# megvii-research/basedet

Hardware: AMD Instinct MI355X
Metric: images/sec training RetinaNet-R50-FPN 1333x800 (higher is better)
Workload: dtype bf16; 1 GPU; retinanet_r50_800x1344 train step (fwd+bwd+allreduce+SGD), DummyLoader boxes, random-init weights, inputs resident in HBM; per_gpu_batch=16, global_batch=16, parallelism=dp1

## Files before the change

### basedet_amd/csrc/gskip.hip

```cpp
#include "common.h"

namespace {

enum { GS_ANY = 1, GS_TOP = 2, GS_BOT = 4, GS_LEFT = 8, GS_RIGHT = 16, GS_TL = 32, GS_TR = 64, GS_BL = 128, GS_BR = 256 };

struct GsSeg { int patch_start, H, W, pw, off; };

struct GsParams {
    const bf16_raw* g;
    int* mask;
    int C, ppi, ph, pw_px, nseg, patches_per_img, total;
    GsSeg seg[BD_MAX_SEGS];
};

__device__ __forceinline__ int gs_level(const GsParams& p, int rem) {
    int s = 0;
#pragma unroll
    for (int k = 1; k < BD_MAX_SEGS; ++k)
        if (k < p.nseg && rem >= p.seg[k].patch_start) s = k;
    return s;
}

__global__ __launch_bounds__(256) void gskip_scan_kernel(const GsParams p) {
    __shared__ int sbits;
    const int tid = threadIdx.x;
    const int pid = blockIdx.x;
    const int n = pid / p.patches_per_img, rem = pid - n * p.patches_per_img;
    const int s = gs_level(p, rem);
    const int H = p.seg[s].H, W = p.seg[s].W, pwn = p.seg[s].pw;
    const int local = rem - p.seg[s].patch_start, by = local / pwn, bx = local - by * pwn;
    const int y0 = by * p.ph, x0 = bx * p.pw_px;
    const int cpp = p.C >> 3;
    const int items = p.ph * p.pw_px * cpp;
    const long long img = (long long)n * p.ppi + p.seg[s].off;
    if (tid == 0) sbits = 0;
    __syncthreads();
    int bits = 0;
    constexpr int U = 8;
    for (int b = 0; b < items; b += 256 * U) {
        u32x4_t v[U];
        int pix[U];
#pragma unroll
        for (int k = 0; k < U; ++k) {
            const int i = b + k * 256 + tid;
            v[k] = (u32x4_t){0u, 0u, 0u, 0u};
            pix[k] = -1;
            if (i < items) {
                const int px = i / cpp, ch = i - px * cpp;
                const int py = px / p.pw_px, pxx = px - py * p.pw_px;
                const int y = y0 + py, x = x0 + pxx;
                if (y < H && x < W) {
                    v[k] = *reinterpret_cast<const u32x4_t*>(p.g + (img + (long long)y * W + x) * p.C + ch * 8);
                    pix[k] = px;
                }
            }
        }
#pragma unroll
        for (int k = 0; k < U; ++k) {
            if (pix[k] >= 0 && (v[k][0] | v[k][1] | v[k][2] | v[k][3])) {
                const int py = pix[k] / p.pw_px, pxx = pix[k] - py * p.pw_px;
                const bool t = py == 0, bo = py == p.ph - 1, l = pxx == 0, r = pxx == p.pw_px - 1;
                bits |= GS_ANY | (t ? GS_TOP : 0) | (bo ? GS_BOT : 0) | (l ? GS_LEFT : 0) | (r ? GS_RIGHT : 0) | (t && l ? GS_TL : 0) |
                        (t && r ? GS_TR : 0) | (bo && l ? GS_BL : 0) | (bo && r ? GS_BR : 0);
            }
        }
    }
#pragma unroll
    for (int m = 32; m >= 1; m >>= 1) bits |= __shfl_xor(bits, m, 64);
    if ((tid & 63) == 0 && bits) atomicOr(&sbits, bits);
    __syncthreads();
    if (tid == 0) p.mask[pid] = sbits;
}

template <bool FRESH>
__device__ __forceinline__ int gs_mask(const int* m, int i) {
    if (FRESH) return __hip_atomic_load(m + i, __ATOMIC_RELAXED, __HIP_MEMORY_SCOPE_AGENT);
    return m[i];
}

template <bool FRESH>
__device__ __forceinline__ void gs_compact_body(const GsParams& p, int* live, int* list, int* count, int* wsum) {
    constexpr int KP = 8;
    const int tid = threadIdx.x, wv = tid >> 6, ln = tid & 63;
    int base = 0;
    for (int c0 = 0; c0 < p.total; c0 += 1024 * KP) {
        int lv[KP];
#pragma unroll
        for (int j = 0; j < KP; ++j) {
            const int q = c0 + tid * KP + j;
            lv[j] = 0;
            if (q < p.total) {
                const int n = q / p.patches_per_img, rem = q - n * p.patches_per_img;
                const int s = gs_level(p, rem);
                const int pwn = p.seg[s].pw, rows = (p.seg[s].H + p.ph - 1) / p.ph;
                const int local = rem - p.seg[s].patch_start, by = local / pwn, bx = local - by * pwn;
                const int* m = p.mask + (long long)n * p.patches_per_img + p.seg[s].patch_start;
                const bool up = by > 0, dn = by + 1 < rows, lf = bx > 0, rt = bx + 1 < pwn;
                int v = gs_mask<FRESH>(m, by * pwn + bx) & GS_ANY;
                if (up) v |= gs_mask<FRESH>(m, (by - 1) * pwn + bx) & GS_BOT;
                if (dn) v |= gs_mask<FRESH>(m, (by + 1) * pwn + bx) & GS_TOP;
                if (lf) v |= gs_mask<FRESH>(m, by * pwn + bx - 1) & GS_RIGHT;
                if (rt) v |= gs_mask<FRESH>(m, by * pwn + bx + 1) & GS_LEFT;
                if (up && lf) v |= gs_mask<FRESH>(m, (by - 1) * pwn + bx - 1) & GS_BR;
                if (up && rt) v |= gs_mask<FRESH>(m, (by - 1) * pwn + bx + 1) & GS_BL;
                if (dn && lf) v |= gs_mask<FRESH>(m, (by + 1) * pwn + bx - 1) & GS_TR;
                if (dn && rt) v |= gs_mask<FRESH>(m, (by + 1) * pwn + bx + 1) & GS_TL;
                lv[j] = v != 0;
            }
        }
        int cnt = 0;
#pragma unroll
        for (int j = 0; j < KP; ++j) cnt += lv[j];
        int inc = cnt;
#pragma unroll
        for (int o = 1; o < 64; o <<= 1) {
            const int y = __shfl_up(inc, o, 64);
            if (ln >= o) inc += y;
        }
        if (ln == 63) wsum[wv] = inc;
        __syncthreads();
        int off = base + inc - cnt, tot = 0;
#pragma unroll
        for (int w = 0; w < 16; ++w) {
            off += w < wv ? wsum[w] : 0;
            tot += wsum[w];
        }
#pragma unroll
        for (int j = 0; j < KP; ++j) {
            const int q = c0 + tid * KP + j;
            if (q < p.total) live[q] = lv[j];
            if (lv[j]) list[off++] = q;
        }
        base += tot;
        __syncthreads();
    }
    if (tid == 0) *count = base;
}

__global__ __launch_bounds__(1024) void gskip_compact_kernel(const GsParams p, int* live, int* list, int* count) {
    __shared__ int wsum[16];
    gs_compact_body<false>(p, live, list, count, wsum);
}

enum { GM_HDR = 8 };

struct GmSeg { int H, W, off, s4, s8, ss; };

struct GmParams {
    const bf16_raw* t;
    const int* live_in;
    int* map;
    int C, ppi, nseg, pi4, pi8, pis, tot4, tot8;
    GmSeg seg[BD_MAX_SEGS];
};

__global__ __launch_bounds__(1024) void gskip_fill_kernel(const GmParams p, const GsParams cp, int total) {
    __shared__ int sbits, slast;
    __shared__ int wsum[16];
    const int tid = threadIdx.x;
    int* m4 = p.map + GM_HDR;
    int* m8 = m4 + p.tot4;
    const int cpp = p.C >> 3;
    const int items = 4 * 16 * cpp;
    for (int pid = blockIdx.x; pid < total; pid += gridDim.x) {
        const int n = pid / p.pis, rem = pid - n * p.pis;
        int s = 0;
#pragma unroll
        for (int k = 1; k < BD_MAX_SEGS; ++k)
            if (k < p.nseg && rem >= p.seg[k].ss) s = k;
        const int H = p.seg[s].H, W = p.seg[s].W;
        const int sc = (W + 15) >> 4, r4 = (H + 3) >> 2, c8 = (W + 7) >> 3;
        const int local = rem - p.seg[s].ss, sy = local / sc, sx = local - sy * sc;
        int q4[2], q8[2];
        bool ok4[2], ok8[2], lv[2];
#pragma unroll
        for (int h = 0; h < 2; ++h) {
            ok4[h] = 2 * sy + h < r4;
            q4[h] = n * p.pi4 + p.seg[s].s4 + (2 * sy + h) * sc + sx;
            ok8[h] = 2 * sx + h < c8;
            q8[h] = n * p.pi8 + p.seg[s].s8 + sy * c8 + 2 * sx + h;
            lv[h] = ok4[h] && (p.live_in == nullptr || p.live_in[q4[h]] != 0);
        }
        int b = 0;
        if (lv[0] || lv[1]) {
            if (tid == 0) sbits = 0;
            __syncthreads();
            const long long img = (long long)n * p.ppi + p.seg[s].off;
            int bits = 0;
#pragma unroll
            for (int h = 0; h < 2; ++h) {
                if (!lv[h]) continue;
                for (int i = tid; i < items; i += 1024) {
                    const int px = i / cpp, ch = i - px * cpp;
                    const int py = px >> 4, pxx = px & 15;
                    const int y = 8 * sy + 4 * h + py, x = 16 * sx + pxx;
                    if (y < H && x < W) {
                        const u32x4_t v = *reinterpret_cast<const u32x4_t*>(p.t + (img + (long long)y * W + x) * p.C + ch * 8);
                        if (v[0] | v[1] | v[2] | v[3]) {
                            const bool t = py == 0, bo = py == 3, l = pxx == 0, r = pxx == 15;
                            const int w = GS_ANY | (t ? GS_TOP : 0) | (bo ? GS_BOT : 0) | (l ? GS_LEFT : 0) | (r ? GS_RIGHT : 0) |
                                          (t && l ? GS_TL : 0) | (t && r ? GS_TR : 0) | (bo && l ? GS_BL : 0) | (bo && r ? GS_BR : 0);
                            bits |= (w << (9 * h)) | (1 << (18 + (pxx >> 3)));
                        }
                    }
                }
            }
#pragma unroll
            for (int m = 32; m >= 1; m >>= 1) bits |= __shfl_xor(bits, m, 64);
            if ((tid & 63) == 0 && bits) atomicOr(&sbits, bits);
            __syncthreads();
            b = sbits;
            __syncthreads();
        }
        if (tid == 0) {
            if (ok4[0]) m4[q4[0]] = b & 511;
            if (ok4[1]) m4[q4[1]] = (b >> 9) & 511;
            if (ok8[0]) m8[q8[0]] = (b >> 18) & 1;
            if (ok8[1]) m8[q8[1]] = (b >> 19) & 1;
        }
    }
    if (tid == 0) {
        __builtin_amdgcn_fence(__ATOMIC_RELEASE, "agent");
        slast = atomicAdd(p.map + 1, 1) == (int)gridDim.x - 1;
    }
    __syncthreads();
    if (!slast) return;
    __builtin_amdgcn_fence(__ATOMIC_ACQUIRE, "agent");
    const int nxt = (p.map[0] & 1) ^ 1;
    int* live = m8 + p.tot8;
    gs_compact_body<true>(cp, live, live + p.tot4 * (1 + nxt), p.map + 2 + nxt, wsum);
    if (tid == 0) { p.map[0] = nxt; p.map[1] = 0; }
}

enum { FL_HDR = 8, FL_MAX_DEPTH = 8 };

struct FlSeg { int H, W, off, s4, pw; };

struct FlParams {
    const int* labels;
    int* map[FL_MAX_DEPTH];
    int A, ppi, nseg, depths, pi4, tot4;
    FlSeg seg[BD_MAX_SEGS];
};

__global__ __launch_bounds__(1024) void fwd_live_kernel(const FlParams p) {
    extern __shared__ __attribute__((aligned(16))) unsigned char fl_bm[];
    __shared__ int slast;
    __shared__ int wsum[16];
    const int tid = threadIdx.x;
    const int n = blockIdx.x / p.nseg, s = blockIdx.x - n * p.nseg;
    const int H = p.seg[s].H, W = p.seg[s].W, HW = H * W, pwn = p.seg[s].pw;
    const int npatch = ((H + 3) >> 2) * pwn;
    unsigned char* cur = fl_bm;
    unsigned char* nxt = fl_bm + HW;
    for (int i = tid; i < HW; i += 1024) cur[i] = 0;
    __syncthreads();
    const int* lab = p.labels + ((long long)n * p.ppi + p.seg[s].off) * p.A;
    for (int i = tid; i < HW * p.A; i += 1024)
        if (lab[i] > 0) cur[i / p.A] = 1;
    __syncthreads();
    for (int k = 0; k < p.depths; ++k) {
        for (int i = tid; i < HW; i += 1024) {
            const int y = i / W, x = i - y * W;
            const int y0 = y > 0 ? y - 1 : 0, y1 = y + 1 < H ? y + 1 : H - 1, x0 = x > 0 ? x - 1 : 0, x1 = x + 1 < W ? x + 1 : W - 1;
            int v = 0;
            for (int yy = y0; yy <= y1; ++yy)
                for (int xx = x0; xx <= x1; ++xx) v |= cur[yy * W + xx];
            nxt[i] = (unsigned char)v;
        }
        __syncthreads();
        int* live = p.map[k] + FL_HDR + n * p.pi4 + p.seg[s].s4;
        for (int q = tid; q < npatch; q += 1024) {
            const int by = q / pwn, bx = q - by * pwn;
            const int ye = by * 4 + 4 < H ? by * 4 + 4 : H, xe = bx * 16 + 16 < W ? bx * 16 + 16 : W;
            int v = 0;
            for (int y = by * 4; y < ye; ++y)
                for (int x = bx * 16; x < xe; ++x) v |= nxt[y * W + x];
            live[q] = v;
        }
        unsigned char* t = cur; cur = nxt; nxt = t;
        __syncthreads();
    }
    __builtin_amdgcn_fence(__ATOMIC_RELEASE, "agent");
    __syncthreads();
    if (tid == 0) slast = atomicAdd(p.map[0] + 1, 1) == (int)gridDim.x - 1;
    __syncthreads();
    if (!slast) return;
    __builtin_amdgcn_fence(__ATOMIC_ACQUIRE, "agent");
    constexpr int KP = 8;
    const int wv = tid >> 6, ln = tid & 63;
    for (int k = 0; k < p.depths; ++k) {
        int* hdr = p.map[k];
        const int* live = hdr + FL_HDR;
        const int to = (hdr[0] & 1) ^ 1;
        int* list = hdr + FL_HDR + p.tot4 * (1 + to);
        int base = 0;
        for (int c0 = 0; c0 < p.tot4; c0 += 1024 * KP) {
            int lv[KP];
            int cnt = 0;
#pragma unroll
            for (int j = 0; j < KP; ++j) {
                const int q = c0 + tid * KP + j;
                lv[j] = q < p.tot4 ? (__hip_atomic_load(live + q, __ATOMIC_RELAXED, __HIP_MEMORY_SCOPE_AGENT) != 0) : 0;
                cnt += lv[j];
            }
            int inc = cnt;
#pragma unroll
            for (int o = 1; o < 64; o <<= 1) {
                const int y = __shfl_up(inc, o, 64);
                if (ln >= o) inc += y;
            }
            if (ln == 63) wsum[wv] = inc;
            __syncthreads();
            int off = base + inc - cnt, tot = 0;
#pragma unroll
            for (int w = 0; w < 16; ++w) {
                off += w < wv ? wsum[w] : 0;
                tot += wsum[w];
            }
#pragma unroll
            for (int j = 0; j < KP; ++j)
                if (lv[j]) list[off++] = c0 + tid * KP + j;
            base += tot;
            __syncthreads();
        }
        if (tid == 0) { hdr[2 + to] = base; hdr[0] = to; }
    }
    if (tid == 0) p.map[0][1] = 0;
}

GsParams gs_params(const bd_conv_desc* d, int ph, int pw, int side = 0) {
    GsParams p{};
    p.C = side ? d->Cin : d->Cout; p.ppi = side ? d->in_pix_per_img : d->out_pix_per_img; p.ph = ph; p.pw_px = pw; p.nseg = d->nseg;
    int ps = 0;
    for (int s = 0; s < d->nseg; ++s) {
        GsSeg& sg = p.seg[s];
        const int H = side ? d->Hi[s] : d->Ho[s], W = side ? d->Wi[s] : d->Wo[s];
        sg.patch_start = ps; sg.H = H; sg.W = W; sg.pw = cdiv(W, pw); sg.off = side ? d->in_off[s] : d->out_off[s];
        ps += cdiv(H, ph) * sg.pw;
    }
    p.patches_per_img = ps;
    p.total = ps * d->N;
    return p;
}

}

int bd_gskip_patches(const bd_conv_desc* d, int ph, int pw) {
    return gs_params(d, ph, pw).total;
}

void bd_gskip_scan(const bd_conv_desc* d, const void* g, int ph, int pw, int* mask, hipStream_t stream) {
    GsParams p = gs_params(d, ph, pw);
    p.g = (const bf16_raw*)g; p.mask = mask;
    if (p.total > 0) hipLaunchKernelGGL(gskip_scan_kernel, dim3(p.total), dim3(256), 0, stream, p);
}

void bd_gskip_compact(const bd_conv_desc* d, int ph, int pw, const int* mask, int* live, int* list, int* count, hipStream_t stream) {
    GsParams p = gs_params(d, ph, pw);
    p.mask = const_cast<int*>(mask);
    hipLaunchKernelGGL(gskip_compact_kernel, dim3(1), dim3(1024), 0, stream, p, live, list, count);
}

void bd_gskip_map_layout(const bd_conv_desc* d, int side, BdGskipMap* out) {
    const int p4 = gs_params(d, 4, 16, side).total, p8 = gs_params(d, 8, 8, side).total;
    out->p4 = p4; out->p8 = p8;
    out->m4 = GM_HDR; out->m8 = GM_HDR + p4; out->live = out->m8 + p8; out->list = out->live + p4;
    out->ints = (size_t)GM_HDR + (size_t)4 * p4 + p8;
}

extern "C" size_t bd_conv2d_gskip_map_bytes(const bd_conv_desc* d, int of_dx) {
    if (!d || d->nseg < 1 || d->nseg > BD_MAX_SEGS || !(d->R == 3 && d->S == 3 && d->stride == 1 && d->pad == 1)) return 0;
    BdGskipMap m;
    bd_gskip_map_layout(d, of_dx ? 1 : 0, &m);
    return m.ints * sizeof(int);
}

void bd_gskip_fill(const bd_conv_desc* d, int side, const void* t, const int* live_in, int* map, hipStream_t stream) {
    const GsParams g4 = gs_params(d, 4, 16, side), g8 = gs_params(d, 8, 8, side), gs = gs_params(d, 8, 16, side);
    GmParams p{};
    p.t = (const bf16_raw*)t; p.live_in = live_in; p.map = map;
    p.C = g4.C; p.ppi = g4.ppi; p.nseg = g4.nseg;
    p.pi4 = g4.patches_per_img; p.pi8 = g8.patches_per_img; p.pis = gs.patches_per_img; p.tot4 = g4.total; p.tot8 = g8.total;
    for (int s = 0; s < g4.nseg; ++s)
        p.seg[s] = GmSeg{g4.seg[s].H, g4.seg[s].W, g4.seg[s].off, g4.seg[s].patch_start, g8.seg[s].patch_start, gs.seg[s].patch_start};
    GsParams cp = g4;
    cp.mask = map + GM_HDR;
    const int grid = gs.total < 128 ? gs.total : 128;
    if (grid > 0) hipLaunchKernelGGL(gskip_fill_kernel, dim3(grid), dim3(1024), 0, stream, p, cp, gs.total);
}

extern "C" int bd_gskip_map_scan(const bd_conv_desc* d, int of_dx, const void* t, void* map, size_t map_bytes, bd_stream_t stream) {
    BD_REQUIRE(d && t && map, "gskip_map_scan: null pointer");
    const size_t need = bd_conv2d_gskip_map_bytes(d, of_dx);
    BD_REQUIRE(need > 0, "gskip_map_scan: liveness maps belong to 3x3 / stride 1 / pad 1 descriptors");
    BD_REQUIRE(map_bytes >= need, "gskip_map_scan: map %zu < required %zu bytes", map_bytes, need);
    const int side = of_dx ? 1 : 0;
    BdGskipMap m;
    bd_gskip_map_layout(d, side, &m);
    int* mp = (int*)map;
    if (hipMemsetAsync(mp, 0, GM_HDR * sizeof(int), (hipStream_t)stream) != hipSuccess) { bd_set_error("gskip_map_scan: memset failed"); return BD_ELAUNCH; }
    GsParams p4 = gs_params(d, 4, 16, side), p8 = gs_params(d, 8, 8, side);
    p4.g = p8.g = (const bf16_raw*)t;
    p4.mask = mp + m.m4; p8.mask = mp + m.m8;
    if (p4.total > 0) {
        hipLaunchKernelGGL(gskip_scan_kernel, dim3(p4.total), dim3(256), 0, (hipStream_t)stream, p4);
        hipLaunchKernelGGL(gskip_scan_kernel, dim3(p8.total), dim3(256), 0, (hipStream_t)stream, p8);
    }
    hipLaunchKernelGGL(gskip_compact_kernel, dim3(1), dim3(1024), 0, (hipStream_t)stream, p4, mp + m.live, mp + m.list, mp + 2);
    BD_CHECK_LAUNCH("bd_gskip_map_scan");
    return BD_OK;
}

void bd_fwd_map_layout(const bd_conv_desc* d, BdFwdMap* out) {
    const int p4 = gs_params(d, 4, 16, 0).total;
    out->p4 = p4; out->live = FL_HDR; out->list = FL_HDR + p4;
    out->ints = (size_t)FL_HDR + (size_t)3 * p4;
}

extern "C" size_t bd_fwd_live_map_bytes(const bd_conv_desc* d) {
    if (!d || d->nseg < 1 || d->nseg > BD_MAX_SEGS || !(d->R == 3 && d->S == 3 && d->stride == 1 && d->pad == 1)) return 0;
    BdFwdMap m;
    bd_fwd_map_layout(d, &m);
    return m.ints * sizeof(int);
}

extern "C" int bd_fwd_live_maps(const bd_conv_desc* d, const int32_t* labels, int A, int depths, void* const* maps, size_t map_bytes,
                                int reset, bd_stream_t stream) {
    BD_REQUIRE(d && labels && maps, "fwd_live_maps: null pointer");
    const size_t need = bd_fwd_live_map_bytes(d);
    BD_REQUIRE(need > 0, "fwd_live_maps: forward liveness maps belong to 3x3 / stride 1 / pad 1 descriptors");
    BD_REQUIRE(A >= 1 && depths >= 1 && depths <= FL_MAX_DEPTH, "fwd_live_maps: A=%d depths=%d (1 .. %d)", A, depths, (int)FL_MAX_DEPTH);
    BD_REQUIRE(map_bytes >= need, "fwd_live_maps: map %zu < required %zu bytes", map_bytes, need);
    const GsParams g4 = gs_params(d, 4, 16, 0);
    FlParams p{};
    p.labels = labels; p.A = A; p.ppi = g4.ppi; p.nseg = g4.nseg; p.depths = depths; p.pi4 = g4.patches_per_img; p.tot4 = g4.total;
    size_t lds = 0;
    for (int s = 0; s < g4.nseg; ++s) {
        BD_REQUIRE(d->Hi[s] == d->Ho[s] && d->Wi[s] == d->Wo[s], "fwd_live_maps: level %d changes size", s);
        p.seg[s] = FlSeg{g4.seg[s].H, g4.seg[s].W, g4.seg[s].off, g4.seg[s].patch_start, g4.seg[s].pw};
        const size_t b = (size_t)2 * g4.seg[s].H * g4.seg[s].W;
        BD_REQUIRE((long long)g4.seg[s].H * g4.seg[s].W * A < 0x7fffffffll, "fwd_live_maps: level %d too large", s);
        lds = b > lds ? b : lds;
    }
    BD_REQUIRE(lds <= 160 * 1024 - 256, "fwd_live_maps: a level of %zu pixels does not fit the LDS bitmap", lds / 2);
    for (int k = 0; k < depths; ++k) {
        BD_REQUIRE(maps[k], "fwd_live_maps: null map %d", k);
        p.map[k] = (int*)maps[k];
        if (reset && hipMemsetAsync(maps[k], 0, FL_HDR * sizeof(int), (hipStream_t)stream) != hipSuccess) {
            bd_set_error("fwd_live_maps: memset failed");
            return BD_ELAUNCH;
        }
    }
    if (d->N < 1 || g4.total < 1) return BD_OK;
    BD_ONCE_PER_DEVICE((void)hipFuncSetAttribute(reinterpret_cast<const void*>(&fwd_live_kernel), hipFuncAttributeMaxDynamicSharedMemorySize,
                                                 160 * 1024 - 256));
    hipLaunchKernelGGL(fwd_live_kernel, dim3(d->N * g4.nseg), dim3(1024), lds, (hipStream_t)stream, p);
    BD_CHECK_LAUNCH("bd_fwd_live_maps");
    return BD_OK;
}
```

Measured before the change: 726.1 images/sec.

## Rework gradient-skip scan, fill and forward-liveness kernels to use wave-level work and bitmaps

```diff
diff --git a/basedet_amd/csrc/gskip.hip b/basedet_amd/csrc/gskip.hip
--- a/basedet_amd/csrc/gskip.hip
+++ b/basedet_amd/csrc/gskip.hip
@@ -21,55 +21,78 @@
     return s;
 }
 
+constexpr int GS_U = 8;
+constexpr int GM_U = 4;
+
+template <int NP>
 __global__ __launch_bounds__(256) void gskip_scan_kernel(const GsParams p) {
-    __shared__ int sbits;
-    const int tid = threadIdx.x;
-    const int pid = blockIdx.x;
-    const int n = pid / p.patches_per_img, rem = pid - n * p.patches_per_img;
-    const int s = gs_level(p, rem);
-    const int H = p.seg[s].H, W = p.seg[s].W, pwn = p.seg[s].pw;
-    const int local = rem - p.seg[s].patch_start, by = local / pwn, bx = local - by * pwn;
-    const int y0 = by * p.ph, x0 = bx * p.pw_px;
+    static_assert(9 * NP <= 31, "the packed GS_* words fit one int");
+    const int lane = threadIdx.x & 63;
+    const int wave = __builtin_amdgcn_readfirstlane(blockIdx.x * 4 + (threadIdx.x >> 6)), nwaves = gridDim.x * 4;
     const int cpp = p.C >> 3;
     const int items = p.ph * p.pw_px * cpp;
-    const long long img = (long long)n * p.ppi + p.seg[s].off;
-    if (tid == 0) sbits = 0;
-    __syncthreads();
-    int bits = 0;
-    constexpr int U = 8;
-    for (int b = 0; b < items; b += 256 * U) {
-        u32x4_t v[U];
-        int pix[U];
-#pragma unroll
-        for (int k = 0; k < U; ++k) {
-            const int i = b + k * 256 + tid;
-            v[k] = (u32x4_t){0u, 0u, 0u, 0u};
-            pix[k] = -1;
-            if (i < items) {
+    const int rows = (items + 63) >> 6;
+    for (int q0 = wave * NP; q0 < p.total; q0 += nwaves * NP) {
+        int H[NP], W[NP], y0[NP], x0[NP];
+        long long img[NP];
+#pragma unroll
+        for (int j = 0; j < NP; ++j) {
+            const int pid = q0 + j < p.total ? q0 + j : p.total - 1;
+            const int n = pid / p.patches_per_img, rem = pid - n * p.patches_per_img;
+            const int s = gs_level(p, rem);
+            const int pwn = p.seg[s].pw;
+            const int local = rem - p.seg[s].patch_start, by = local / pwn, bx = local - by * pwn;
+            H[j] = q0 + j < p.total ? p.seg[s].H : 0;
+            W[j] = p.seg[s].W;
+            y0[j] = by * p.ph; x0[j] = bx * p.pw_px;
+            img[j] = (long long)n * p.ppi + p.seg[s].off;
+        }
+        int bits = 0;
+        for (int b = 0; b < rows; b += GS_U) {
+            u32x4_t v[NP][GS_U];
+            int pix[GS_U];
+#pragma unroll
+            for (int k = 0; k < GS_U; ++k) {
+                const int i = (b + k) * 64 + lane;
                 const int px = i / cpp, ch = i - px * cpp;
                 const int py = px / p.pw_px, pxx = px - py * p.pw_px;
-                const int y = y0 + py, x = x0 + pxx;
-                if (y < H && x < W) {
-                    v[k] = *reinterpret_cast<const u32x4_t*>(p.g + (img + (long long)y * W + x) * p.C + ch * 8);
-                    pix[k] = px;
+                pix[k] = i < items ? px : -1;
+#pragma unroll
+                for (int j = 0; j < NP; ++j) {
+                    const int y = y0[j] + py, x = x0[j] + pxx;
+                    v[j][k] = (u32x4_t){0u, 0u, 0u, 0u};
+                    if (i < items && y < H[j] && x < W[j])
+                        v[j][k] = *reinterpret_cast<const u32x4_t*>(p.g + (img[j] + (long long)y * W[j] + x) * p.C + ch * 8);
                 }
             }
-        }
-#pragma unroll
-        for (int k = 0; k < U; ++k) {
-            if (pix[k] >= 0 && (v[k][0] | v[k][1] | v[k][2] | v[k][3])) {
+#pragma unroll
+            for (int k = 0; k < GS_U; ++k) {
+                if (pix[k] < 0) continue;
                 const int py = pix[k] / p.pw_px, pxx = pix[k] - py * p.pw_px;
                 const bool t = py == 0, bo = py == p.ph - 1, l = pxx == 0, r = pxx == p.pw_px - 1;
-                bits |= GS_ANY | (t ? GS_TOP : 0) | (bo ? GS_BOT : 0) | (l ? GS_LEFT : 0) | (r ? GS_RIGHT : 0) | (t && l ? GS_TL : 0) |
-                        (t && r ? GS_TR : 0) | (bo && l ? GS_BL : 0) | (bo && r ? GS_BR : 0);
-            }
-        }
-    }
-#pragma unroll
-    for (int m = 32; m >= 1; m >>= 1) bits |= __shfl_xor(bits, m, 64);
-    if ((tid & 63) == 0 && bits) atomicOr(&sbits, bits);
-    __syncthreads();
-    if (tid == 0) p.mask[pid] = sbits;
+                const int w = GS_ANY | (t ? GS_TOP : 0) | (bo ? GS_BOT : 0) | (l ? GS_LEFT : 0) | (r ? GS_RIGHT : 0) | (t && l ? GS_TL : 0) |
+                              (t && r ? GS_TR : 0) | (bo && l ? GS_BL : 0) | (bo && r ? GS_BR : 0);
+#pragma unroll
+                for (int j = 0; j < NP; ++j)
+                    if (v[j][k][0] | v[j][k][1] | v[j][k][2] | v[j][k][3]) bits |= w << (9 * j);
+            }
+        }
+#pragma unroll
+        for (int m = 32; m >= 1; m >>= 1) bits |= __shfl_xor(bits, m, 64);
+        if (lane == 0) {
+#pragma unroll
+            for (int j = 0; j < NP; ++j)
+                if (q0 + j < p.total) p.mask[q0 + j] = (bits >> (9 * j)) & 511;
+        }
+    }
+}
+
+void gs_launch_scan(const GsParams& p, hipStream_t stream) {
+    if (p.total < 1) return;
+    const bool thin = (p.C >> 3) <= GS_U;
+    const int np = thin ? 2 : 1, need = cdiv(cdiv(p.total, np), 4), grid = need < 4096 ? need : 4096;
+    if (thin) hipLaunchKernelGGL(gskip_scan_kernel<2>, dim3(grid), dim3(256), 0, stream, p);
+    else hipLaunchKernelGGL(gskip_scan_kernel<1>, dim3(grid), dim3(256), 0, stream, p);
 }
 
 template <bool FRESH>
@@ -154,70 +177,108 @@
     GmSeg seg[BD_MAX_SEGS];
 };
 
+struct GmBlock {
+    int H, W, sy, sx, q4[2], q8[2];
+    bool ok4[2], ok8[2];
+    long long img;
+};
+
+__device__ __forceinline__ GmBlock gm_block(const GmParams& p, int pid) {
+    GmBlock k;
+    const int n = pid / p.pis, rem = pid - n * p.pis;
+    int s = 0;
+#pragma unroll
+    for (int j = 1; j < BD_MAX_SEGS; ++j)
+        if (j < p.nseg && rem >= p.seg[j].ss) s = j;
+    k.H = p.seg[s].H; k.W = p.seg[s].W;
+    const int sc = (k.W + 15) >> 4, r4 = (k.H + 3) >> 2, c8 = (k.W + 7) >> 3;
+    const int local = rem - p.seg[s].ss;
+    k.sy = local / sc; k.sx = local - k.sy * sc;
+#pragma unroll
+    for (int h = 0; h < 2; ++h) {
+        k.ok4[h] = 2 * k.sy + h < r4;
+        k.q4[h] = n * p.pi4 + p.seg[s].s4 + (2 * k.sy + h) * sc + k.sx;
+        k.ok8[h] = 2 * k.sx + h < c8;
+        k.q8[h] = n * p.pi8 + p.seg[s].s8 + k.sy * c8 + 2 * k.sx + h;
+    }
+    k.img = (long long)n * p.ppi + p.seg[s].off;
+    return k;
+}
+
+__device__ __forceinline__ void gm_store(int* m4, int* m8, const GmBlock& k, int b) {
+    if (k.ok4[0]) m4[k.q4[0]] = b & 511;
+    if (k.ok4[1]) m4[k.q4[1]] = (b >> 9) & 511;
+    if (k.ok8[0]) m8[k.q8[0]] = (b >> 18) & 1;
+    if (k.ok8[1]) m8[k.q8[1]] = (b >> 19) & 1;
+}
+
 __global__ __launch_bounds__(1024) void gskip_fill_kernel(const GmParams p, const GsParams cp, int total) {
-    __shared__ int sbits, slast;
+    __shared__ int slast, scount;
     __shared__ int wsum[16];
-    const int tid = threadIdx.x;
+    __shared__ int slist[1024];
+    const int tid = threadIdx.x, wv = tid >> 6, lane = tid & 63;
     int* m4 = p.map + GM_HDR;
     int* m8 = m4 + p.tot4;
     const int cpp = p.C >> 3;
-    const int items = 4 * 16 * cpp;
-    for (int pid = blockIdx.x; pid < total; pid += gridDim.x) {
-        const int n = pid / p.pis, rem = pid - n * p.pis;
-        int s = 0;
-#pragma unroll
-        for (int k = 1; k < BD_MAX_SEGS; ++k)
-            if (k < p.nseg && rem >= p.seg[k].ss) s = k;
-        const int H = p.seg[s].H, W = p.seg[s].W;
-        const int sc = (W + 15) >> 4, r4 = (H + 3) >> 2, c8 = (W + 7) >> 3;
-        const int local = rem - p.seg[s].ss, sy = local / sc, sx = local - sy * sc;
-        int q4[2], q8[2];
-        bool ok4[2], ok8[2], lv[2];
-#pragma unroll
-        for (int h = 0; h < 2; ++h) {
-            ok4[h] = 2 * sy + h < r4;
-            q4[h] = n * p.pi4 + p.seg[s].s4 + (2 * sy + h) * sc + sx;
-            ok8[h] = 2 * sx + h < c8;
-            q8[h] = n * p.pi8 + p.seg[s].s8 + sy * c8 + 2 * sx + h;
-            lv[h] = ok4[h] && (p.live_in == nullptr || p.live_in[q4[h]] != 0);
-        }
-        int b = 0;
-        if (lv[0] || lv[1]) {
-            if (tid == 0) sbits = 0;
-            __syncthreads();
-            const long long img = (long long)n * p.ppi + p.seg[s].off;
+    for (int r0 = 0; blockIdx.x + (long long)r0 * gridDim.x < total; r0 += 1024) {
+        if (tid == 0) scount = 0;
+        __syncthreads();
+        {
+            const long long pl = blockIdx.x + (long long)(r0 + tid) * gridDim.x;
+            int code = 0;
+            if (pl < total) {
+                const int pid = (int)pl;
+                const GmBlock k = gm_block(p, pid);
+                const bool lv0 = k.ok4[0] && (p.live_in == nullptr || p.live_in[k.q4[0]] != 0);
+                const bool lv1 = k.ok4[1] && (p.live_in == nullptr || p.live_in[k.q4[1]] != 0);
+                if (lv0 || lv1) code = pid * 4 + (lv0 ? 1 : 0) + (lv1 ? 2 : 0);
+                else gm_store(m4, m8, k, 0);
+            }
+            const unsigned long long bal = __ballot(code != 0);
+            int base = 0;
+            if (lane == 0 && bal) base = atomicAdd(&scount, __popcll(bal));
+            base = __shfl(base, 0, 64);
+            if (code) slist[base + __popcll(bal & ((1ull << lane) - 1))] = code;
+        }
+        __syncthreads();
+        const int nlive = scount;
+        for (int e = wv; e < nlive; e += 16) {
+            const int code = slist[e];
+            const GmBlock k = gm_block(p, code >> 2);
             int bits = 0;
-#pragma unroll
-            for (int h = 0; h < 2; ++h) {
-                if (!lv[h]) continue;
-                for (int i = tid; i < items; i += 1024) {
+            for (int c0 = 0; c0 < cpp; c0 += GM_U) {
+                u32x4_t v[2][GM_U];
+#pragma unroll
+                for (int u = 0; u < GM_U; ++u) {
+                    const int i = (c0 + u) * 64 + lane;
                     const int px = i / cpp, ch = i - px * cpp;
                     const int py = px >> 4, pxx = px & 15;
-                    const int y = 8 * sy + 4 * h + py, x = 16 * sx + pxx;
-                    if (y < H && x < W) {
-                        const u32x4_t v = *reinterpret_cast<const u32x4_t*>(p.t + (img + (long long)y * W + x) * p.C + ch * 8);
-                        if (v[0] | v[1] | v[2] | v[3]) {
-                            const bool t = py == 0, bo = py == 3, l = pxx == 0, r = pxx == 15;
-                            const int w = GS_ANY | (t ? GS_TOP : 0) | (bo ? GS_BOT : 0) | (l ? GS_LEFT : 0) | (r ? GS_RIGHT : 0) |
-                                          (t && l ? GS_TL : 0) | (t && r ? GS_TR : 0) | (bo && l ? GS_BL : 0) | (bo && r ? GS_BR : 0);
-                            bits |= (w << (9 * h)) | (1 << (18 + (pxx >> 3)));
-                        }
+                    const int x = 16 * k.sx + pxx;
+#pragma unroll
+                    for (int h = 0; h < 2; ++h) {
+                        const int y = 8 * k.sy + 4 * h + py;
+                        v[h][u] = (u32x4_t){0u, 0u, 0u, 0u};
+                        if (c0 + u < cpp && ((code >> h) & 1) && y < k.H && x < k.W)
+                            v[h][u] = *reinterpret_cast<const u32x4_t*>(p.t + (k.img + (long long)y * k.W + x) * p.C + ch * 8);
                     }
                 }
+#pragma unroll
+                for (int u = 0; u < GM_U; ++u) {
+                    const int px = ((c0 + u) * 64 + lane) / cpp;
+                    const int py = px >> 4, pxx = px & 15;
+                    const bool t = py == 0, bo = py == 3, l = pxx == 0, r = pxx == 15;
+                    const int w = GS_ANY | (t ? GS_TOP : 0) | (bo ? GS_BOT : 0) | (l ? GS_LEFT : 0) | (r ? GS_RIGHT : 0) |
+                                  (t && l ? GS_TL : 0) | (t && r ? GS_TR : 0) | (bo && l ? GS_BL : 0) | (bo && r ? GS_BR : 0);
+#pragma unroll
+                    for (int h = 0; h < 2; ++h)
+                        if (v[h][u][0] | v[h][u][1] | v[h][u][2] | v[h][u][3]) bits |= (w << (9 * h)) | (1 << (18 + (pxx >> 3)));
+                }
             }
 #pragma unroll
             for (int m = 32; m >= 1; m >>= 1) bits |= __shfl_xor(bits, m, 64);
-            if ((tid & 63) == 0 && bits) atomicOr(&sbits, bits);
-            __syncthreads();
-            b = sbits;
-            __syncthreads();
-        }
-        if (tid == 0) {
-            if (ok4[0]) m4[q4[0]] = b & 511;
-            if (ok4[1]) m4[q4[1]] = (b >> 9) & 511;
-            if (ok8[0]) m8[q8[0]] = (b >> 18) & 1;
-            if (ok8[1]) m8[q8[1]] = (b >> 19) & 1;
-        }
+            if (lane == 0) gm_store(m4, m8, k, bits);
+        }
+        __syncthreads();
     }
     if (tid == 0) {
         __builtin_amdgcn_fence(__ATOMIC_RELEASE, "agent");
@@ -243,52 +304,83 @@
     FlSeg seg[BD_MAX_SEGS];
 };
 
+constexpr int FL_T = 4, FL_AU = 9;
+
+__host__ __device__ __forceinline__ int fl_words_per_row(int W) { return (W + 63) >> 6; }
+
 __global__ __launch_bounds__(1024) void fwd_live_kernel(const FlParams p) {
-    extern __shared__ __attribute__((aligned(16))) unsigned char fl_bm[];
+    extern __shared__ __attribute__((aligned(16))) unsigned long long fl_bm[];
     __shared__ int slast;
     __shared__ int wsum[16];
-    const int tid = threadIdx.x;
+    const int tid = threadIdx.x, wv = tid >> 6, lane = tid & 63;
     const int n = blockIdx.x / p.nseg, s = blockIdx.x - n * p.nseg;
-    const int H = p.seg[s].H, W = p.seg[s].W, HW = H * W, pwn = p.seg[s].pw;
+    const int H = p.seg[s].H, W = p.seg[s].W, pwn = p.seg[s].pw;
+    const int wpr = fl_words_per_row(W), nw = H * wpr;
     const int npatch = ((H + 3) >> 2) * pwn;
-    unsigned char* cur = fl_bm;
-    unsigned char* nxt = fl_bm + HW;
-    for (int i = tid; i < HW; i += 1024) cur[i] = 0;
+    unsigned long long* cur = fl_bm;
+    unsigned long long* nxt = fl_bm + nw;
+    const int* lab = p.labels + ((long long)n * p.ppi + p.seg[s].off) * p.A;
+    for (int t0 = wv * FL_T; t0 < nw; t0 += 16 * FL_T) {
+        bool fg[FL_T];
+#pragma unroll
+        for (int j = 0; j < FL_T; ++j) fg[j] = false;
+        for (int a0 = 0; a0 < p.A; a0 += FL_AU) {
+            int v[FL_T][FL_AU];
+#pragma unroll
+            for (int j = 0; j < FL_T; ++j) {
+                const int t = t0 + j, y = t / wpr, x = (t - y * wpr) * 64 + lane;
+                const bool ok = t < nw && x < W;
+#pragma unroll
+                for (int a = 0; a < FL_AU; ++a) v[j][a] = ok && a0 + a < p.A ? lab[(y * W + x) * p.A + a0 + a] : 0;
+            }
+#pragma unroll
+            for (int j = 0; j < FL_T; ++j)
+#pragma unroll
+                for (int a = 0; a < FL_AU; ++a) fg[j] = fg[j] || v[j][a] > 0;
+        }
+#pragma unroll
+        for (int j = 0; j < FL_T; ++j) {
+            const unsigned long long w = __ballot(fg[j]);
+            if (lane == 0 && t0 + j < nw) cur[t0 + j] = w;
+        }
+    }
     __syncthreads();
-    const int* lab = p.labels + ((long long)n * p.ppi + p.seg[s].off) * p.A;
-    for (int i = tid; i < HW * p.A; i += 1024)
-        if (lab[i] > 0) cur[i / p.A] = 1;
-    __syncthreads();
+    const unsigned long long last = (W & 63) ? (1ull << (W & 63)) - 1 : ~0ull;
     for (int k = 0; k < p.depths; ++k) {
-        for (int i = tid; i < HW; i += 1024) {
-            const int y = i / W, x = i - y * W;
-            const int y0 = y > 0 ? y - 1 : 0, y1 = y + 1 < H ? y + 1 : H - 1, x0 = x > 0 ? x - 1 : 0, x1 = x + 1 < W ? x + 1 : W - 1;
-            int v = 0;
-            for (int yy = y0; yy <= y1; ++yy)
-                for (int xx = x0; xx <= x1; ++xx) v |= cur[yy * W + xx];
-            nxt[i] = (unsigned char)v;
+        for (int i = tid; i < nw; i += 1024) {
+            const int y = i / wpr, wx = i - y * wpr;
+            const int y0 = y > 0 ? y - 1 : 0, y1 = y + 1 < H ? y + 1 : H - 1;
+            unsigned long long o = 0;
+            for (int yy = y0; yy <= y1; ++yy) {
+                const unsigned long long* r = cur + yy * wpr;
+                const unsigned long long w = r[wx];
+                o |= w | (w << 1) | (w >> 1);
+                if (wx > 0) o |= r[wx - 1] >> 63;
+                if (wx + 1 < wpr) o |= r[wx + 1] << 63;
+            }
+            nxt[i] = wx == wpr - 1 ? o & last : o;
         }
         __syncthreads();
         int* live = p.map[k] + FL_HDR + n * p.pi4 + p.seg[s].s4;
         for (int q = tid; q < npatch; q += 1024) {
             const int by = q / pwn, bx = q - by * pwn;
-            const int ye = by * 4 + 4 < H ? by * 4 + 4 : H, xe = bx * 16 + 16 < W ? bx * 16 + 16 : W;
-            int v = 0;
-            for (int y = by * 4; y < ye; ++y)
-                for (int x = bx * 16; x < xe; ++x) v |= nxt[y * W + x];
-            live[q] = v;
-        }
-        unsigned char* t = cur; cur = nxt; nxt = t;
-        __syncthreads();
-    }
-    __builtin_amdgcn_fence(__ATOMIC_RELEASE, "agent");
+            const int ye = by * 4 + 4 < H ? by * 4 + 4 : H;
+            unsigned long long v = 0;
+            for (int y = by * 4; y < ye; ++y) v |= nxt[y * wpr + (bx >> 2)];
+            live[q] = ((v >> ((bx & 3) * 16)) & 0xffffull) != 0;
+        }
+        unsigned long long* t = cur; cur = nxt; nxt = t;
+    }
     __syncthreads();
-    if (tid == 0) slast = atomicAdd(p.map[0] + 1, 1) == (int)gridDim.x - 1;
+    if (tid == 0) {
+        __builtin_amdgcn_fence(__ATOMIC_RELEASE, "agent");
+        slast = atomicAdd(p.map[0] + 1, 1) == (int)gridDim.x - 1;
+    }
     __syncthreads();
     if (!slast) return;
     __builtin_amdgcn_fence(__ATOMIC_ACQUIRE, "agent");
     constexpr int KP = 8;
-    const int wv = tid >> 6, ln = tid & 63;
+    const int ln = lane;
     for (int k = 0; k < p.depths; ++k) {
         int* hdr = p.map[k];
         const int* live = hdr + FL_HDR;
@@ -353,7 +445,7 @@
 void bd_gskip_scan(const bd_conv_desc* d, const void* g, int ph, int pw, int* mask, hipStream_t stream) {
     GsParams p = gs_params(d, ph, pw);
     p.g = (const bf16_raw*)g; p.mask = mask;
-    if (p.total > 0) hipLaunchKernelGGL(gskip_scan_kernel, dim3(p.total), dim3(256), 0, stream, p);
+    gs_launch_scan(p, stream);
 }
 
 void bd_gskip_compact(const bd_conv_desc* d, int ph, int pw, const int* mask, int* live, int* list, int* count, hipStream_t stream) {
@@ -403,10 +495,8 @@
     GsParams p4 = gs_params(d, 4, 16, side), p8 = gs_params(d, 8, 8, side);
     p4.g = p8.g = (const bf16_raw*)t;
     p4.mask = mp + m.m4; p8.mask = mp + m.m8;
-    if (p4.total > 0) {
-        hipLaunchKernelGGL(gskip_scan_kernel, dim3(p4.total), dim3(256), 0, (hipStream_t)stream, p4);
-        hipLaunchKernelGGL(gskip_scan_kernel, dim3(p8.total), dim3(256), 0, (hipStream_t)stream, p8);
-    }
+    gs_launch_scan(p4, (hipStream_t)stream);
+    gs_launch_scan(p8, (hipStream_t)stream);
     hipLaunchKernelGGL(gskip_compact_kernel, dim3(1), dim3(1024), 0, (hipStream_t)stream, p4, mp + m.live, mp + m.list, mp + 2);
     BD_CHECK_LAUNCH("bd_gskip_map_scan");
     return BD_OK;
@@ -439,11 +529,11 @@
     for (int s = 0; s < g4.nseg; ++s) {
         BD_REQUIRE(d->Hi[s] == d->Ho[s] && d->Wi[s] == d->Wo[s], "fwd_live_maps: level %d changes size", s);
         p.seg[s] = FlSeg{g4.seg[s].H, g4.seg[s].W, g4.seg[s].off, g4.seg[s].patch_start, g4.seg[s].pw};
-        const size_t b = (size_t)2 * g4.seg[s].H * g4.seg[s].W;
+        const size_t b = (size_t)2 * g4.seg[s].H * fl_words_per_row(g4.seg[s].W) * sizeof(unsigned long long);
         BD_REQUIRE((long long)g4.seg[s].H * g4.seg[s].W * A < 0x7fffffffll, "fwd_live_maps: level %d too large", s);
         lds = b > lds ? b : lds;
     }
-    BD_REQUIRE(lds <= 160 * 1024 - 256, "fwd_live_maps: a level of %zu pixels does not fit the LDS bitmap", lds / 2);
+    BD_REQUIRE(lds <= 160 * 1024 - 256, "fwd_live_maps: a level's bitmap of %zu bytes does not fit the LDS", lds / 2);
     for (int k = 0; k < depths; ++k) {
         BD_REQUIRE(maps[k], "fwd_live_maps: null map %d", k);
         p.map[k] = (int*)maps[k];
```

Result: no change. 730.4 images/sec, median of 6 (+0.6%).

## Map gskip patches to single wavefronts and batch fill-kernel liveness work

Applied to the files above, without the earlier changes.

```diff
diff --git a/basedet_amd/csrc/gskip.hip b/basedet_amd/csrc/gskip.hip
--- a/basedet_amd/csrc/gskip.hip
+++ b/basedet_amd/csrc/gskip.hip
@@ -70,6 +70,51 @@
     if ((tid & 63) == 0 && bits) atomicOr(&sbits, bits);
     __syncthreads();
     if (tid == 0) p.mask[pid] = sbits;
+}
+
+__global__ __launch_bounds__(256) void gskip_scan_narrow_kernel(const GsParams p) {
+    const int ln = threadIdx.x & 63;
+    const int pid = blockIdx.x * 4 + (threadIdx.x >> 6);
+    if (pid >= p.total) return;
+    const int n = pid / p.patches_per_img, rem = pid - n * p.patches_per_img;
+    const int s = gs_level(p, rem);
+    const int H = p.seg[s].H, W = p.seg[s].W, pwn = p.seg[s].pw;
+    const int local = rem - p.seg[s].patch_start, by = local / pwn, bx = local - by * pwn;
+    const int y0 = by * p.ph, x0 = bx * p.pw_px;
+    const int cpp = p.C >> 3;
+    const int npx = p.ph * p.pw_px;
+    const long long img = (long long)n * p.ppi + p.seg[s].off;
+    int bits = 0;
+    for (int px = ln; px < npx; px += 64) {
+        const int py = px / p.pw_px, pxx = px - py * p.pw_px;
+        const int y = y0 + py, x = x0 + pxx;
+        if (y < H && x < W) {
+            const u32x4_t* src = reinterpret_cast<const u32x4_t*>(p.g + (img + (long long)y * W + x) * p.C);
+            u32x4_t v[8];
+#pragma unroll
+            for (int c = 0; c < 8; ++c) {
+                v[c] = (u32x4_t){0u, 0u, 0u, 0u};
+                if (c < cpp) v[c] = src[c];
+            }
+            unsigned any = 0;
+#pragma unroll
+            for (int c = 0; c < 8; ++c) any |= v[c][0] | v[c][1] | v[c][2] | v[c][3];
+            if (any) {
+                const bool t = py == 0, bo = py == p.ph - 1, l = pxx == 0, r = pxx == p.pw_px - 1;
+                bits |= GS_ANY | (t ? GS_TOP : 0) | (bo ? GS_BOT : 0) | (l ? GS_LEFT : 0) | (r ? GS_RIGHT : 0) | (t && l ? GS_TL : 0) |
+                        (t && r ? GS_TR : 0) | (bo && l ? GS_BL : 0) | (bo && r ? GS_BR : 0);
+            }
+        }
+    }
+#pragma unroll
+    for (int m = 32; m >= 1; m >>= 1) bits |= __shfl_xor(bits, m, 64);
+    if (ln == 0) p.mask[pid] = bits;
+}
+
+void gs_launch_scan(const GsParams& p, hipStream_t stream) {
+    if (p.total < 1) return;
+    if (p.C <= 64) hipLaunchKernelGGL(gskip_scan_narrow_kernel, dim3(cdiv(p.total, 4)), dim3(256), 0, stream, p);
+    else hipLaunchKernelGGL(gskip_scan_kernel, dim3(p.total), dim3(256), 0, stream, p);
 }
 
 template <bool FRESH>
@@ -154,74 +199,104 @@
     GmSeg seg[BD_MAX_SEGS];
 };
 
+__device__ __forceinline__ void gm_block(const GmParams& p, int pid, int& n, int& s, int& sy, int& sx) {
+    n = pid / p.pis;
+    const int rem = pid - n * p.pis;
+    s = 0;
+#pragma unroll
+    for (int k = 1; k < BD_MAX_SEGS; ++k)
+        if (k < p.nseg && rem >= p.seg[k].ss) s = k;
+    const int sc = (p.seg[s].W + 15) >> 4;
+    const int local = rem - p.seg[s].ss;
+    sy = local / sc;
+    sx = local - sy * sc;
+}
+
 __global__ __launch_bounds__(1024) void gskip_fill_kernel(const GmParams p, const GsParams cp, int total) {
-    __shared__ int sbits, slast;
+    __shared__ int sidx[4 * 1024];
+    __shared__ int sres[2 * 1024];
+    __shared__ int slive[2 * 1024];
+    __shared__ int snl, slast;
     __shared__ int wsum[16];
-    const int tid = threadIdx.x;
+    const int tid = threadIdx.x, wv = tid >> 6, ln = tid & 63;
     int* m4 = p.map + GM_HDR;
     int* m8 = m4 + p.tot4;
     const int cpp = p.C >> 3;
     const int items = 4 * 16 * cpp;
-    for (int pid = blockIdx.x; pid < total; pid += gridDim.x) {
-        const int n = pid / p.pis, rem = pid - n * p.pis;
-        int s = 0;
-#pragma unroll
-        for (int k = 1; k < BD_MAX_SEGS; ++k)
-            if (k < p.nseg && rem >= p.seg[k].ss) s = k;
-        const int H = p.seg[s].H, W = p.seg[s].W;
-        const int sc = (W + 15) >> 4, r4 = (H + 3) >> 2, c8 = (W + 7) >> 3;
-        const int local = rem - p.seg[s].ss, sy = local / sc, sx = local - sy * sc;
-        int q4[2], q8[2];
-        bool ok4[2], ok8[2], lv[2];
-#pragma unroll
-        for (int h = 0; h < 2; ++h) {
-            ok4[h] = 2 * sy + h < r4;
-            q4[h] = n * p.pi4 + p.seg[s].s4 + (2 * sy + h) * sc + sx;
-            ok8[h] = 2 * sx + h < c8;
-            q8[h] = n * p.pi8 + p.seg[s].s8 + sy * c8 + 2 * sx + h;
-            lv[h] = ok4[h] && (p.live_in == nullptr || p.live_in[q4[h]] != 0);
-        }
-        int b = 0;
-        if (lv[0] || lv[1]) {
-            if (tid == 0) sbits = 0;
-            __syncthreads();
+    const int per = (total - (int)blockIdx.x + (int)gridDim.x - 1) / (int)gridDim.x;
+    for (int k0 = 0; k0 < per; k0 += 1024) {
+        if (tid == 0) snl = 0;
+        __syncthreads();
+        if (k0 + tid < per) {
+            int n, s, sy, sx;
+            gm_block(p, blockIdx.x + (k0 + tid) * gridDim.x, n, s, sy, sx);
+            const int sc = (p.seg[s].W + 15) >> 4, r4 = (p.seg[s].H + 3) >> 2, c8 = (p.seg[s].W + 7) >> 3;
+#pragma unroll
+            for (int h = 0; h < 2; ++h) {
+                const bool ok4 = 2 * sy + h < r4, ok8 = 2 * sx + h < c8;
+                const int q4 = n * p.pi4 + p.seg[s].s4 + (2 * sy + h) * sc + sx;
+                const int q8 = n * p.pi8 + p.seg[s].s8 + sy * c8 + 2 * sx + h;
+                sidx[4 * tid + h] = ok4 ? q4 : -1;
+                sidx[4 * tid + 2 + h] = ok8 ? p.tot4 + q8 : -1;
+                sres[2 * tid + h] = 0;
+                if (ok4 && (p.live_in == nullptr || p.live_in[q4] != 0)) slive[atomicAdd(&snl, 1)] = 2 * tid + h;
+            }
+        }
+        __syncthreads();
+        const int nl = snl;
+        for (int j = wv; j < nl; j += 16) {
+            const int e = slive[j], h = e & 1;
+            int n, s, sy, sx;
+            gm_block(p, blockIdx.x + (k0 + (e >> 1)) * gridDim.x, n, s, sy, sx);
+            const int H = p.seg[s].H, W = p.seg[s].W;
             const long long img = (long long)n * p.ppi + p.seg[s].off;
             int bits = 0;
-#pragma unroll
-            for (int h = 0; h < 2; ++h) {
-                if (!lv[h]) continue;
-                for (int i = tid; i < items; i += 1024) {
-                    const int px = i / cpp, ch = i - px * cpp;
-                    const int py = px >> 4, pxx = px & 15;
-                    const int y = 8 * sy + 4 * h + py, x = 16 * sx + pxx;
-                    if (y < H && x < W) {
-                        const u32x4_t v = *reinterpret_cast<const u32x4_t*>(p.t + (img + (long long)y * W + x) * p.C + ch * 8);
-                        if (v[0] | v[1] | v[2] | v[3]) {
-                            const bool t = py == 0, bo = py == 3, l = pxx == 0, r = pxx == 15;
-                            const int w = GS_ANY | (t ? GS_TOP : 0) | (bo ? GS_BOT : 0) | (l ? GS_LEFT : 0) | (r ? GS_RIGHT : 0) |
-                                          (t && l ? GS_TL : 0) | (t && r ? GS_TR : 0) | (bo && l ? GS_BL : 0) | (bo && r ? GS_BR : 0);
-                            bits |= (w << (9 * h)) | (1 << (18 + (pxx >> 3)));
+            constexpr int U = 8;
+            for (int b = 0; b < items; b += 64 * U) {
+                u32x4_t v[U];
+                int pix[U];
+#pragma unroll
+                for (int k = 0; k < U; ++k) {
+                    const int i = b + k * 64 + ln;
+                    v[k] = (u32x4_t){0u, 0u, 0u, 0u};
+                    pix[k] = -1;
+                    if (i < items) {
+                        const int px = i / cpp, ch = i - px * cpp;
+                        const int y = 8 * sy + 4 * h + (px >> 4), x = 16 * sx + (px & 15);
+                        if (y < H && x < W) {
+                            v[k] = *reinterpret_cast<const u32x4_t*>(p.t + (img + (long long)y * W + x) * p.C + ch * 8);
+                            pix[k] = px;
                         }
                     }
                 }
+#pragma unroll
+                for (int k = 0; k < U; ++k) {
+                    if (pix[k] >= 0 && (v[k][0] | v[k][1] | v[k][2] | v[k][3])) {
+                        const int py = pix[k] >> 4, pxx = pix[k] & 15;
+                        const bool t = py == 0, bo = py == 3, l = pxx == 0, r = pxx == 15;
+                        bits |= GS_ANY | (t ? GS_TOP : 0) | (bo ? GS_BOT : 0) | (l ? GS_LEFT : 0) | (r ? GS_RIGHT : 0) | (t && l ? GS_TL : 0) |
+                                (t && r ? GS_TR : 0) | (bo && l ? GS_BL : 0) | (bo && r ? GS_BR : 0) | (1 << (9 + (pxx >> 3)));
+                    }
+                }
             }
 #pragma unroll
             for (int m = 32; m >= 1; m >>= 1) bits |= __shfl_xor(bits, m, 64);
-            if ((tid & 63) == 0 && bits) atomicOr(&sbits, bits);
-            __syncthreads();
-            b = sbits;
-            __syncthreads();
-        }
-        if (tid == 0) {
-            if (ok4[0]) m4[q4[0]] = b & 511;
-            if (ok4[1]) m4[q4[1]] = (b >> 9) & 511;
-            if (ok8[0]) m8[q8[0]] = (b >> 18) & 1;
-            if (ok8[1]) m8[q8[1]] = (b >> 19) & 1;
-        }
-    }
-    if (tid == 0) {
+            if (ln == 0) sres[e] = bits;
+        }
+        __syncthreads();
+        if (wv == 0) {
+            const int nb = per - k0 < 1024 ? per - k0 : 1024;
+            for (int e = ln; e < 4 * nb; e += 64) {
+                const int at = sidx[e], w = e & 3;
+                const int r0 = sres[2 * (e >> 2)], r1 = sres[2 * (e >> 2) + 1];
+                if (at >= 0) m4[at] = w == 0 ? r0 & 511 : w == 1 ? r1 & 511 : ((r0 | r1) >> (7 + w)) & 1;
+            }
+        }
+        __syncthreads();
+    }
+    if (wv == 0) {
         __builtin_amdgcn_fence(__ATOMIC_RELEASE, "agent");
-        slast = atomicAdd(p.map + 1, 1) == (int)gridDim.x - 1;
+        if (tid == 0) slast = atomicAdd(p.map + 1, 1) == (int)gridDim.x - 1;
     }
     __syncthreads();
     if (!slast) return;
@@ -353,7 +428,7 @@
 void bd_gskip_scan(const bd_conv_desc* d, const void* g, int ph, int pw, int* mask, hipStream_t stream) {
     GsParams p = gs_params(d, ph, pw);
     p.g = (const bf16_raw*)g; p.mask = mask;
-    if (p.total > 0) hipLaunchKernelGGL(gskip_scan_kernel, dim3(p.total), dim3(256), 0, stream, p);
+    gs_launch_scan(p, stream);
 }
 
 void bd_gskip_compact(const bd_conv_desc* d, int ph, int pw, const int* mask, int* live, int* list, int* count, hipStream_t stream) {
@@ -403,10 +478,8 @@
     GsParams p4 = gs_params(d, 4, 16, side), p8 = gs_params(d, 8, 8, side);
     p4.g = p8.g = (const bf16_raw*)t;
     p4.mask = mp + m.m4; p8.mask = mp + m.m8;
-    if (p4.total > 0) {
-        hipLaunchKernelGGL(gskip_scan_kernel, dim3(p4.total), dim3(256), 0, (hipStream_t)stream, p4);
-        hipLaunchKernelGGL(gskip_scan_kernel, dim3(p8.total), dim3(256), 0, (hipStream_t)stream, p8);
-    }
+    gs_launch_scan(p4, (hipStream_t)stream);
+    gs_launch_scan(p8, (hipStream_t)stream);
     hipLaunchKernelGGL(gskip_compact_kernel, dim3(1), dim3(1024), 0, (hipStream_t)stream, p4, mp + m.live, mp + m.list, mp + 2);
     BD_CHECK_LAUNCH("bd_gskip_map_scan");
     return BD_OK;
```

Result: no change. 722.3 images/sec before, 726.0 images/sec after (median of 6 runs) (+0.5%).
